# MrGiovanni/R-Super

Hardware: AMD Instinct MI355X
Metric: CT voxels/sec/node (96³ patch, bs=2/GPU) (higher is better)
Workload: dtype bf16; 1 GPU; R-Super 3D UNet(base 32, 26 classes, BasicBlock/IN) full training step (fwd + masked BCE + Dice loss + bwd + clip + AdamW + EMA), 96^3 patches, batch 2/GPU (BASELINE.json configs[1]); global_batch=2, patch=96, parallelism=dp1, sanity_checks_form=device-side flags read one step late (train_ddp.StepGuard)

## Files before the change

include/rsuper_hip.h:

```cpp
#ifndef RSUPER_HIP_H
#define RSUPER_HIP_H
#include <stddef.h>
#include <stdint.h>
#ifdef __cplusplus
extern "C" {
#endif

#define RSUPER_F32 0
#define RSUPER_BF16 1
#define RSUPER_OK 0
#define RSUPER_ERR_ARG 1
#define RSUPER_ERR_LAUNCH 2
#define RSUPER_ERR_UNSUPPORTED 3
#define RSUPER_ERR_NO_DEVICE 4

const char* rsuper_version(void);
int rsuper_device_check(void);


size_t rsuper_conv3_packed_elems(int dtype, int ka, int kb, int n_cols, int bn);

int rsuper_conv3_pack_weights(int dtype, int mode, const float* wa, const float* wb, int ka, int kb, int na, int nb,
                              int bn, void* packed, void* stream);

int rsuper_conv3_pack_weights_batch(int dtype, int n, const int* host_desc, const float* const* host_wa, const float* const* host_wb,
                                    const size_t* host_out_elems, void* packed, void* stream);

int rsuper_conv3_tiles(int D, int H, int W);

int rsuper_conv3_variant(int v);
int rsuper_conv3_wgrad2_min_tiles(int t);

int rsuper_conv3_plan(int dtype, int epi, int N, int D, int H, int W, int Ca, int Cb, int n_cols, int src_flags, int bn, int* plan);

int rsuper_conv3_box_bn(int dtype, int N, int D, int H, int W, int n_cols);

int rsuper_conv3_kd_bn(int dtype, int epi, int N, int D, int H, int W, int n_cols, int src_flags);

int rsuper_conv3_set_workspace(void* ptr, size_t bytes);
size_t rsuper_conv3_workspace_bytes(void);

int rsuper_conv3_part_rows(int dtype, int epi, int N, int D, int H, int W, int n_cols, int bn, int src_flags);

int rsuper_conv3_igemm(int dtype, int epi,
                       const void* xa, int lda, int Ca, const float* mra,
                       const void* xb, int ldb, int Cb, const float* mrb,
                       const void* packed, int n_cols, int bn, int N, int D, int H, int W,
                       void* out, int ldo, const void* res, int ldr, float* part,
                       const void* exa, int elda, int eCa, const float* emra,
                       const void* exb, int eldb, int eCb, const float* emrb, void* stream);
int rsuper_conv3_igemm_split_out(int dtype, int epi,
                                 const void* xa, int lda, int Ca, const float* mra,
                                 const void* xb, int ldb, int Cb, const float* mrb,
                                 const void* packed, int n_cols, int bn, int N, int D, int H, int W,
                                 void* out, int ldo, const void* res, int ldr, float* part,
                                 const void* exa, int elda, int eCa, const float* emra,
                                 const void* exb, int eldb, int eCb, const float* emrb, int out_split, long long out_part, void* stream);
int rsuper_conv3_s2_part_rows(int dtype, int mode, int Ca, int Cb, int n_cols, int N, int FD, int FH, int FW);
int rsuper_conv3_igemm_s2(int dtype, int mode, const void* xa, int lda, int Ca, const float* mra,
                          const void* xb, int ldb, int Cb, const void* packed, int n_cols, int N, int FD, int FH, int FW,
                          void* out, int ldo, float* part, const void* exa, int elda, const float* emra, void* stream);

int rsuper_conv3_wgrad_splits(int dtype, int Ca, int Cb, int Ya, int Yb, int N, int D, int H, int W);

// ... 219 lines not shown
```

r-super_amd/csrc/api.hip:

```cpp
#include <string.h>
#include <math.h>
#include <stdlib.h>
#include "common.hpp"
#include "kernels.hpp"
#include "misc.hpp"
#include "loss.hpp"
#include "morph.hpp"
#include "optim.hpp"
#include "../../include/rsuper_hip.h"

#define ST(s) ((hipStream_t)(s))

static inline bool dt_ok(int dt) { return dt == RS_F32 || dt == RS_BF16; }
static inline bool ch_ok(int C, int ld) { return C >= 0 && (C % 8) == 0 && (ld % 8) == 0 && ld >= C; }
static inline bool bn_ok(int bn) { return bn == 32 || bn == 64 || bn == 96 || bn == 128; }
static inline int ntiles_for(int n_cols, int bn) { const int per = bn / 32; return ((n_cols + bn - 1) / bn) * per; }
static inline int pack_cols(int mode, int na, int nb) { return mode == 1 ? (nb ? (nb & 0xFFFF) : na) : na + nb; }
static inline bool pack_range_ok(int mode, int na, int nb) { return mode != 1 || nb == 0 || ((nb >> 16) % 32 == 0 && (nb & 0xFFFF) > 0 && (nb >> 16) + (nb & 0xFFFF) <= na); }

#include "igemm_plan.hpp"

template <typename F>
static int for_chunks(int n, void* const* p, void* const* g, void* const* m, void* const* v, void* const* e, const size_t* numel, F f) {
    for (int i0 = 0; i0 < n; i0 += RS_MT_MAX) {
// ... 53 lines not shown
                                    const size_t* host_out_elems, void* packed, void* stream) {
    if (!dt_ok(dtype) || n <= 0 || !host_desc || !host_wa || !host_wb || !host_out_elems || !packed) return RS_ERR_ARG;
    const int KP = dtype == RS_F32 ? 4 : 8;
    for (int i0 = 0; i0 < n; i0 += RS_PACK_BATCH_MAX) {
        PackBatch b;
        memset(&b, 0, sizeof(b));
        b.n = n - i0 < RS_PACK_BATCH_MAX ? n - i0 : RS_PACK_BATCH_MAX;
        const size_t base = host_out_elems[i0];
        for (int i = 0; i < b.n; ++i) {
            const int* d = host_desc + (size_t)(i0 + i) * 6;
            if ((d[0] != 0 && d[0] != 1) || d[1] <= 0 || d[2] < 0 || d[3] <= 0 || d[4] < 0 || !bn_ok(d[5])) return RS_ERR_ARG;
            PackParams& q = b.q[i];
            q.wa = host_wa[i0 + i]; q.wb = host_wb[i0 + i]; q.mode = d[0]; q.ka = d[1]; q.kb = d[2]; q.na = d[3]; q.nb = d[4];
            if (!pack_range_ok(d[0], d[3], d[4])) return RS_ERR_ARG;
            q.ntiles = ntiles_for(pack_cols(d[0], d[3], d[4]), d[5]);
            if (!q.wa || ((host_out_elems[i0 + i] - base) % KP)) return RS_ERR_ARG;
            b.vec_start[i] = (host_out_elems[i0 + i] - base) / KP;
        }
        const int* dl = host_desc + (size_t)(i0 + b.n - 1) * 6;
        b.vec_start[b.n] = b.vec_start[b.n - 1] + rs_packed_elems(dtype, dl[1], dl[2], ntiles_for(pack_cols(dl[0], dl[3], dl[4]), dl[5])) / KP;
        for (int i = 0; i + 1 < b.n; ++i) {
            const int* d = host_desc + (size_t)(i0 + i) * 6;
            if (b.vec_start[i] + rs_packed_elems(dtype, d[1], d[2], ntiles_for(pack_cols(d[0], d[3], d[4]), d[5])) / KP != b.vec_start[i + 1]) return RS_ERR_ARG;
        }
        const int rc = rs_launch_pack_batch(b, dtype, (char*)packed + base * (dtype == RS_F32 ? 4 : 2), ST(stream));
        if (rc) return rc;
    }
    return RS_OK;
}

int rsuper_conv3_tiles(int D, int H, int W) { return ((D + 3) / 4) * ((H + 3) / 4) * ((W + 15) / 16); }

int rsuper_conv3_wgrad2_min_tiles(int t) { return rs_wgrad2_min_tiles(t); }

int rsuper_conv3_variant(int v) {
    if (v >= 0 && v <= 8 && v != 5) g_variant = v;
    return g_variant;
}
int rsuper_conv3_plan(int dtype, int epi, int N, int D, int H, int W, int Ca, int Cb, int n_cols, int src_flags, int bn, int* plan) {
    const IgemmPlan pl = igemm_plan(dtype, epi, N, D, H, W, Ca, Cb, n_cols, src_flags, bn);
    if (!plan || pl.kernel < 0) return RS_ERR_ARG;
    plan[0] = pl.kernel; plan[1] = pl.bn; plan[2] = pl.box_cfg; plan[3] = pl.nsplit; plan[4] = pl.part_rows;
    return RS_OK;
}
int rsuper_conv3_kd_bn(int dtype, int epi, int N, int D, int H, int W, int n_cols, int src_flags) {
    const IgemmPlan pl = igemm_plan(dtype, epi, N, D, H, W, 0, 0, n_cols, src_flags, 0);
    return pl.kernel == RS_IGEMM_KD ? pl.bn : 0;
}
int rsuper_conv3_box_bn(int dtype, int N, int D, int H, int W, int n_cols) {
    const IgemmPlan pl = igemm_plan(dtype, 0, N, D, H, W, 0, 0, n_cols, 1, 0);
    return pl.kernel == RS_IGEMM_BOX ? pl.bn : 0;
}
int rsuper_conv3_part_rows(int dtype, int epi, int N, int D, int H, int W, int n_cols, int bn, int src_flags) {
    return bn ? igemm_plan(dtype, epi, N, D, H, W, 0, 0, n_cols, src_flags, bn).part_rows : 0;
}

int rsuper_conv3_set_workspace(void* ptr, size_t bytes) {
    g_ws = ptr; g_ws_bytes = ptr ? bytes : 0;
    return RS_OK;
}
size_t rsuper_conv3_workspace_bytes(void) { return BOXC_WS_BYTES; }

int rsuper_conv3_s2_part_rows(int dtype, int mode, int Ca, int Cb, int n_cols, int N, int FD, int FH, int FW) {
    if ((mode != 1 && mode != 2) || FD <= 0 || FH <= 0 || FW <= 0 || N <= 0 || n_cols <= 0) return 0;
    const int OD = (FD + 1) / 2, OH = (FH + 1) / 2, OW = (FW + 1) / 2, td = mode == 2 ? 2 : 4;
    const S2Kernel k = s2_kernel(dtype, mode, Ca, Cb, n_cols, N, FD, FH, FW);
// ... 649 lines not shown
```

r-super_amd/csrc/conv3d_wgrad2.hip:

```cpp
#include "common.hpp"
#include "kernels.hpp"
#include "wgrad_frag.hpp"
#include <stdio.h>
#include <stdlib.h>
#include <type_traits>

namespace {

#ifdef WG2_PROF
__device__ unsigned long long g_wg2_prof[8 * 4];
#endif

constexpr int TD = 4, TH = 4, TW = 16, HD = TD + 2, HH = TH + 2, HW = TW + 2;
constexpr int XROWS = HD * HH * HW;
constexpr int XBYTES = XROWS * 64;
constexpr int YPLANE = 256 * 64;
constexpr int NT = 512, NW = 8;

__device__ __forceinline__ void dma16(const __amdgpu_buffer_rsrc_t& rs, uint32_t voff, uint32_t lds_byte) {
    asm volatile("s_mov_b32 m0, %1\n\ts_nop 0\n\tbuffer_load_dwordx4 %0, %2, 0 offen lds" : : "v"(voff), "s"(lds_byte), "s"(rs) : "memory", "m0");
}

constexpr bool pair_in_group(int G, int pidx) { return G < 3 ? pidx < 7 : pidx >= 7; }
constexpr bool unit_valid(int NDL, int dp, int hp, int pidx) {
    const int d = dp - pidx / 3, h = hp - pidx % 3;
    return d >= 0 && d < NDL && h >= 0 && h < TH;
}
constexpr int frag_uses(int G, int NDL, int dp, int hp) {
    int n = 0;
    for (int pidx = 0; pidx < 9; ++pidx) n += (pair_in_group(G, pidx) && unit_valid(NDL, dp, hp, pidx)) ? 1 : 0;
    return n;
}
struct Sched { int n; int dp[64], hp[64], kw[64]; };
constexpr Sched make_sched(int G, int NDL) {
    Sched s{};
    for (int dp = 0; dp < NDL + 2; ++dp)
        for (int hp = 0; hp < HH; ++hp) {
            if (frag_uses(G, NDL, dp, hp) == 0) continue;
            for (int kw = (G < 3 ? G : 0); kw <= (G < 3 ? G : 2); ++kw) { s.dp[s.n] = dp; s.hp[s.n] = hp; s.kw[s.n] = kw; ++s.n; }
        }
    return s;
}

template <int MT, int BD, bool NORM>
__global__ __launch_bounds__(NT, 2) void wgrad2_kernel(WgradParams p) {
    constexpr int NDL = MT == 2 ? 4 : 2;
    constexpr int BUF = XBYTES + MT * YPLANE;
    constexpr int NXV = (XROWS * 4 + NT - 1) / NT;
    constexpr int YK = 16 * MT / NW;
    constexpr int NV = NXV;
    extern __shared__ __attribute__((aligned(16))) char smem[];

    const int tid = threadIdx.x, lane = tid & 63;
    const int wave = __builtin_amdgcn_readfirstlane(tid >> 6);
    const int wsel = wave & 1, g = wave >> 1;
    const int dsel = MT == 1 ? wsel * 2 : 0;
    const int tiles_w = (p.W + TW - 1) / TW, tiles_h = (p.H + TH - 1) / TH, tiles_d = (p.D + TD - 1) / TD;
    const int tiles_per_sample = tiles_w * tiles_h * tiles_d;
    const WgBlockMap bm = wg_block_map(tiles_per_sample * p.N, p.splits);
    const int nchA = (p.xa.C + 31) / 32;
    const bool isB = bm.bx >= nchA;
    const ConvSrc& xs = isB ? p.xb : p.xa;
    const int c0 = (isB ? bm.bx - nchA : bm.bx) * 32;
    const int cin_total = p.xa.C + p.xb.C;
    const int cin_base = (isB ? p.xa.C : 0) + c0;
    const int Mtot = p.ya.C + p.yb.C;
    const int m0 = bm.by * MT * 32;
    constexpr bool norm = NORM;
    const int tiles = tiles_per_sample * p.N;

    const int x_off = dsel * (HH * HW * 64) + frag_lane_off<1>(64, lane);
    const int ya_off = XBYTES + (MT == 2 ? wsel * YPLANE : 0) + dsel * (TH * TW * 64) + frag_lane_off<1>(64, lane);

    const int s_slot = tid & 3, s_row = tid >> 2;
    const uint32_t nvox_total = (uint32_t)(p.N * p.D * p.H * p.W);
    const uint32_t xrowb = (uint32_t)xs.ld * 2u;
    const __amdgpu_buffer_rsrc_t xrs = __builtin_amdgcn_make_buffer_rsrc((void*)xs.x, 0, nvox_total * xrowb, 0x00020000);
    uint32_t xoffb[NXV], xpm[NXV];
    const bool x_cok = c0 + s_slot * 8 < xs.C;
#pragma unroll
    for (int i = 0; i < NXV; ++i) {
        const int r = s_row + 128 * i;
        const int hd = r / (HH * HW), rem = r - hd * (HH * HW);
        const int hh = rem / HW, hw = rem - hh * HW;
        xoffb[i] = (uint32_t)((hd * p.H + hh) * p.W + hw) * xrowb + (uint32_t)(c0 + s_slot * 8) * 2u;
        xpm[i] = (r < XROWS && x_cok) ? ((1u << hd) | (1u << (6 + hh)) | (1u << (12 + hw))) : (1u << 31);
    }
    const int x_st = s_row * 64 + s_slot * 16;
    const int prow = lane >> 2, pslot = lane & 3;
    __amdgpu_buffer_rsrc_t yrs[MT];
    uint32_t yrowb[MT], yoffb[MT];
    bool yok[MT];
#pragma unroll
    for (int q = 0; q < MT; ++q) {
        const int mq = m0 + 32 * q;
        const bool inA = mq < p.ya.C;
        const ConvSrc& ys = inA ? p.ya : p.yb;
        const int ch = (inA ? mq : mq - p.ya.C) + pslot * 8;
        yok[q] = mq < Mtot && ch < ys.C;
        yrowb[q] = (uint32_t)ys.ld * 2u;
        yoffb[q] = (uint32_t)prow * yrowb[q] + (uint32_t)ch * 2u;
        yrs[q] = __builtin_amdgcn_make_buffer_rsrc((void*)ys.x, 0, nvox_total * yrowb[q], 0x00020000);
    }
    const uint32_t lds0 = (uint32_t)(uintptr_t)(__attribute__((address_space(3))) char*)smem;
    const uint32_t ywbit = 1u << (8 + prow);

    const int tile0 = bm.tile0, tile_end = bm.tile_end, tstride = bm.tstride;

    struct IssueTile { uint32_t baseb, ybase; uint32_t xbad, ybad; int n; };
    uint4* dtab = (uint4*)(smem + 2 * BUF + p.N * 256);
    const int ntile = tile0 < tile_end ? (tile_end - 1 - tile0) / tstride + 1 : 0;
    for (int k = tid; k < ntile + 3; k += NT) {
        const bool live = k < ntile;
        const int q = live ? tile0 + k * tstride : 0;
        const int n = q / tiles_per_sample;
        int tw, th, td;
        rs_tile_coords(q - n * tiles_per_sample, tiles_w, tiles_h, tiles_d, tw, th, td);
        const int d0 = td * TD, h0 = th * TH, w0 = tw * TW;
        auto range = [](int o, int len, int nh) {
            const int lo = o >= 0 ? 0 : -o;
            int hi_ = len - 1 - o; if (hi_ > nh - 1) hi_ = nh - 1;
            return hi_ < lo ? 0u : (((2u << hi_) - 1u) & ~((1u << lo) - 1u));
        };
        const uint32_t xbad = live ? ~(range(d0 - 1, p.D, HD) | (range(h0 - 1, p.H, HH) << 6) | (range(w0 - 1, p.W, HW) << 12)) : 0xFFFFFFFFu;
        const uint32_t ybad = live ? (~(range(d0, p.D, TD) | (range(h0, p.H, TH) << 4) | (range(w0, p.W, TW) << 8)) & 0xFFFFFFu) : 0xFFFFFFu;
        dtab[k] = make_uint4((uint32_t)(((n * p.D + d0 - 1) * p.H + (h0 - 1)) * p.W + (w0 - 1)) * xrowb,
                             (uint32_t)(((n * p.D + d0) * p.H + h0) * p.W + w0), xbad, ybad | ((uint32_t)n << 24));
    }
    auto fetch_desc = [&](int k) {
        const uint4 v = dtab[k];
        IssueTile t;
        t.baseb = __builtin_amdgcn_readfirstlane(v.x); t.ybase = __builtin_amdgcn_readfirstlane(v.y);
        t.xbad = __builtin_amdgcn_readfirstlane(v.z);
        const uint32_t w = __builtin_amdgcn_readfirstlane(v.w);
        t.ybad = w & 0xFFFFFFu; t.n = (int)(w >> 24);
        return t;
    };
    uint4 px[NXV];
    auto ld16 = [&](const __amdgpu_buffer_rsrc_t& rs, uint32_t off) {
        const auto q = __builtin_amdgcn_raw_buffer_load_b128(rs, off, 0, 0);
        return make_uint4(q[0], q[1], q[2], q[3]);
    };
    auto issue_v = [&](const IssueTile& t, int i) {
        const bool ok = (xpm[i] & t.xbad) == 0u;
        px[i] = ld16(xrs, ok ? t.baseb + xoffb[i] : 0xFFFFFFF0u);
    };
    auto dma_y = [&](const IssueTile& t, int k, uint32_t buf) {
        const int y = wave + NW * k;
        const int q = MT == 1 ? 0 : (y >> 4), line = y & 15, d = line >> 2, h = line & 3;
        const uint32_t lbit = (1u << d) | (1u << (4 + h)) | ywbit;
        const bool ok = yok[q] && (lbit & t.ybad) == 0u;
        const uint32_t voff = ok ? (t.ybase + (uint32_t)((d * p.H + h) * p.W)) * yrowb[q] + yoffb[q] : 0xFFFFFFF0u;
        dma16(MT == 1 ? yrs[0] : (q ? yrs[MT - 1] : yrs[0]), voff, lds0 + buf + XBYTES + (uint32_t)y * 1024u);
    };
    float4* ntab = (float4*)(smem + 2 * BUF);
    if (norm) {
        for (int e = tid; e < p.N * 16; e += NT) {
            const int n = e >> 4, c = c0 + (e & 15) * 2;
            float4 v = make_float4(1.f, 1.f, 0.f, 0.f);
            if (c < xs.C) { const float* m = xs.mr + ((size_t)n * xs.C + c) * 2; v = make_float4(m[1], m[3], -m[0] * m[1], -m[2] * m[3]); }
            ntab[e] = v;
        }
    }
    const float4* nrow = ntab + s_slot * 4;
    float4 ncst[4];
    int cur_n = -1;
    auto load_norm = [&](int n) {
        if (!norm || n == cur_n) return;
        cur_n = n;
#pragma unroll
        for (int j = 0; j < 4; ++j) ncst[j] = nrow[16 * n + j];
    };
    auto commit_v = [&](char* buf, int i, const IssueTile& t) {
        {
            uint4 q = px[i];
            if (norm) {
                const uint32_t w[4] = {q.x, q.y, q.z, q.w};
                uint32_t o[4];
                const uint32_t m = (xpm[i] & t.xbad) == 0u ? 0xFFFFFFFFu : 0u;
#pragma unroll
                for (int j = 0; j < 4; ++j) {
                    const float4 c = ncst[j];
#ifndef WG2_PKFMA
                    float x0, x1;
                    asm("v_fma_f32 %0, %1, %2, %3" : "=v"(x0) : "v"(__uint_as_float(w[j] << 16)), "v"(c.x), "v"(c.z));
                    asm("v_fma_f32 %0, %1, %2, %3" : "=v"(x1) : "v"(__uint_as_float(w[j] & 0xffff0000u)), "v"(c.y), "v"(c.w));
                    i16x2_t v = __builtin_bit_cast(i16x2_t, f2bf2(x0, x1));
#else
                    f32x2_t x = {__uint_as_float(w[j] << 16), __uint_as_float(w[j] & 0xffff0000u)};
                    const f32x2_t s2 = {c.x, c.y}, b2 = {c.z, c.w};
                    x = __builtin_elementwise_fma(x, s2, b2);
                    i16x2_t v = __builtin_bit_cast(i16x2_t, f2bf2(x[0], x[1]));
#endif
                    const i16x2_t z = {0, 0};
                    v = __builtin_elementwise_max(v, z);
                    o[j] = __builtin_bit_cast(uint32_t, v) & m;
                }
                q = make_uint4(o[0], o[1], o[2], o[3]);
            }
            if (s_row + 128 * i < XROWS) *(uint4*)(buf + x_st + i * 8192) = q;
        }
    };

    auto run = [&](auto G_) {
        constexpr int G = std::remove_reference_t<decltype(G_)>::value;
        constexpr Sched S = make_sched(G, NDL);
        constexpr int KDMIN = G < 3 ? 0 : 2;
        constexpr int AP = NDL < 3 ? NDL : 3;
#ifndef WG2_HOOK_MODE
#define WG2_HOOK_MODE 1
#endif
        constexpr int HMODE = WG2_HOOK_MODE;
        constexpr bool late = HMODE == 0 ? false : ((G < 2) == (HMODE == 1));
        auto hook_step = [&](int i) constexpr { return HMODE == 0 ? (i * S.n) / NV : (late ? S.n / 2 : 0) + (i * (S.n / 2)) / NV; };
        f32x16_t acc[7];
#pragma unroll
        for (int i = 0; i < 7; ++i)
#pragma unroll
            for (int r = 0; r < 16; ++r) acc[i][r] = 0.f;

        __syncthreads();
        IssueTile t1 = fetch_desc(1);
        {
            const IssueTile t0 = fetch_desc(0);
#pragma unroll
            for (int k = 0; k < YK; ++k) dma_y(t0, k, 0);
#pragma unroll
            for (int i = 0; i < NV; ++i) issue_v(t0, i);
            load_norm(t0.n);
#pragma unroll
            for (int i = 0; i < NV; ++i) commit_v(smem, i, t0);
#pragma unroll
            for (int i = 0; i < NV; ++i) issue_v(t1, i);
        }
        asm volatile("s_waitcnt vmcnt(%0)" : : "n"(NV) : "memory");
        __syncthreads();

#ifdef WG2_PROF
        unsigned long long pf_loop = 0, pf_bar = 0;
#endif
        int it = 0;
        for (int tile = tile0; tile < tile_end; tile += tstride, ++it) {
#ifdef WG2_PROF
            const unsigned long long q0 = __builtin_readcyclecounter();
#endif
            const char* buf = smem + (it & 1) * BUF;
            char* nxt = smem + ((it + 1) & 1) * BUF;
            const IssueTile t2 = fetch_desc(it + 2);
            load_norm(t1.n);
#ifndef WG2_SKIP_STAGE
#pragma unroll
            for (int k = 0; k < YK; ++k) dma_y(t1, k, (uint32_t)((it + 1) & 1) * BUF);
#endif
            auto fetch_a = [&](int row) { return frag_bf16<1>(buf + ya_off + (row * TW) * 64, 64); };
            auto fetch_b = [&](int s) { return frag_bf16<1>(buf + x_off + ((S.dp[s] * HH + S.hp[s]) * HW + S.kw[s]) * 64, 64); };
            constexpr int BR = BD + 1;
            uint4 a[AP * TH], bq[BR];
#pragma unroll
            for (int h = 0; h < TH; ++h) a[h] = fetch_a(h);
#pragma unroll
            for (int s = 0; s < BD; ++s) bq[s] = fetch_b(s);
#pragma unroll
            for (int s = 0; s < S.n; ++s) {
#ifndef WG2_PRIO
#define WG2_PRIO 1
#endif
                if (WG2_PRIO == 1) {
                    if (s == 0) __builtin_amdgcn_s_setprio(3);
                    if (s == S.n / 4) __builtin_amdgcn_s_setprio(2);
                    if (s == S.n / 2) __builtin_amdgcn_s_setprio(1);
                    if (s == (3 * S.n) / 4) __builtin_amdgcn_s_setprio(0);
                }
                if (s + BD < S.n) bq[(s + BD) % BR] = fetch_b(s + BD);
                {
                    constexpr bool ring = AP < NDL;
                    const int pl = S.dp[s] - KDMIN + 1;
                    const bool first_of_plane = s == 0 || S.dp[s] != S.dp[s - 1];
                    const bool first_hp4 = S.hp[s] >= 4 && (s == 0 || S.dp[s] != S.dp[s - 1] || S.hp[s - 1] < 4);
                    if (pl >= 1 && pl < NDL && ((ring && G < 3) ? first_hp4 : first_of_plane)) {
#pragma unroll
                        for (int h = 0; h < TH; ++h) a[(pl % AP) * TH + h] = fetch_a(pl * TH + h);
                    }
                }
                __builtin_amdgcn_sched_barrier(0);
#pragma unroll
                for (int pidx = 0; pidx < 9; ++pidx) {
                    if (!pair_in_group(G, pidx) || !unit_valid(NDL, S.dp[s], S.hp[s], pidx)) continue;
                    const int d = S.dp[s] - pidx / 3, h = S.hp[s] - pidx % 3;
                    const int slot = G < 3 ? pidx : (pidx - 7) * 3 + S.kw[s];
#ifndef WG2_SKIP_MMA
                    mma32<bf16_t>(acc[slot], a[(d % AP) * TH + h], bq[s % BR]);
#else
                    if (s == 0) mma32<bf16_t>(acc[slot], a[(d % AP) * TH + h], bq[s % BR]);
#endif
                }
#ifndef WG2_SKIP_STAGE
#pragma unroll
                for (int i = 0; i < NV; ++i)
                    if (s == hook_step(i)) { commit_v(nxt, i, t1); issue_v(t2, i); }
#endif
                __builtin_amdgcn_sched_barrier(0);
            }
#ifdef WG2_PROF
            const unsigned long long q1 = __builtin_readcyclecounter();
#endif
#ifndef WG2_SKIP_STAGE
            asm volatile("s_waitcnt vmcnt(%0)" : : "n"(NV) : "memory");
#endif
            __syncthreads();
#ifdef WG2_PROF
            const unsigned long long q2 = __builtin_readcyclecounter();
            pf_loop += q1 - q0; pf_bar += q2 - q1;
#endif
            t1 = t2;
        }

#ifdef WG2_PROF
        if (blockIdx.x == 0 && blockIdx.y == 0 && blockIdx.z == 0 && lane == 0) { g_wg2_prof[wave * 4] = pf_loop; g_wg2_prof[wave * 4 + 1] = pf_bar; g_wg2_prof[wave * 4 + 2] = (unsigned long long)it; }
#endif
        if constexpr (MT == 1) {
            float* red = (float*)smem + (size_t)g * 7 * 16 * 64 + lane;
            if (wsel == 1) {
#pragma unroll
                for (int i = 0; i < 7; ++i)
#pragma unroll
                    for (int r = 0; r < 16; ++r) red[(i * 16 + r) * 64] = acc[i][r];
            }
            __syncthreads();
            if (wsel == 0) {
#pragma unroll
                for (int i = 0; i < 7; ++i)
#pragma unroll
                    for (int r = 0; r < 16; ++r) acc[i][r] += red[(i * 16 + r) * 64];
            }
        }
        if (MT == 2 || wsel == 0) {
            const int ci = c0 + (lane & 31);
            float* slab = p.ws + (size_t)bm.bz * 27 * Mtot * cin_total;
            const int mrow0 = m0 + (MT == 2 ? wsel * 32 : 0);
#pragma unroll
            for (int i = 0; i < (G < 3 ? 7 : 6); ++i) {
                const int tap = G < 3 ? i * 3 + G : 21 + i;
#pragma unroll
                for (int r = 0; r < 16; ++r) {
                    const int m = mrow0 + cd_row32(r, lane);
                    if (m < Mtot && ci < xs.C) slab[((size_t)tap * Mtot + m) * cin_total + cin_base + (lane & 31)] = acc[i][r];
                }
            }
        }
    };
    switch (g) {
        case 0: run(std::integral_constant<int, 0>{}); break;
        case 1: run(std::integral_constant<int, 1>{}); break;
        case 2: run(std::integral_constant<int, 2>{}); break;
        default: run(std::integral_constant<int, 3>{}); break;
    }
}

template <int MT, int BD, bool NORM>
int launch2(const WgradParams& p, hipStream_t st) {
    const int tiles = p.N * ((p.D + TD - 1) / TD) * ((p.H + TH - 1) / TH) * ((p.W + TW - 1) / TW);
    const int smem = 2 * (XBYTES + MT * YPLANE) + p.N * 256 + ((tiles + p.splits - 1) / p.splits + 4) * 16;
    if (smem > 160 * 1024) return RS_ERR_UNSUPPORTED;
    static_assert(MT == 2 || 4 * 7 * 16 * 64 * 4 <= 2 * (XBYTES + MT * YPLANE), "depth-half reduction scratch must fit the tile buffers");
    const int nch = (p.xa.C + 31) / 32 + (p.xb.C + 31) / 32;
    const int Mtot = p.ya.C + p.yb.C;
    dim3 grid(nch, (Mtot + MT * 32 - 1) / (MT * 32), p.splits), block(NT);
    auto k = wgrad2_kernel<MT, BD, NORM>;
    (void)hipFuncSetAttribute((const void*)k, hipFuncAttributeMaxDynamicSharedMemorySize, smem);
    hipLaunchKernelGGL(k, grid, block, smem, st, p);
#ifdef WG2_PROF
    if (getenv("RSUPER_WG2_PROF")) {
        unsigned long long h[32];
        (void)hipDeviceSynchronize();
        (void)hipMemcpyFromSymbol(h, HIP_SYMBOL(g_wg2_prof), sizeof(h));
        fprintf(stderr, "wg2_prof MT%d norm%d:", MT, (int)NORM);
        for (int w = 0; w < 8; ++w) fprintf(stderr, " w%d(g%d) loop %.0f bar %.0f |", w, w >> 1, (double)h[w * 4] / h[w * 4 + 2], (double)h[w * 4 + 1] / h[w * 4 + 2]);
        fprintf(stderr, " tiles %llu\n", h[2]);
    }
#endif
    return RS_OK;
}

}

bool rs_wgrad2_supported(const WgradParams& p, int dtype) {
    static const int off = getenv("RSUPER_WGRAD2") ? atoi(getenv("RSUPER_WGRAD2")) == 0 : 0;
    if (off || dtype != RS_BF16 || p.N > 32) return false;
    if (p.yb.C > 0 && (p.ya.C % 32)) return false;
    if ((p.xa.mr != nullptr) != (p.xb.C > 0 ? p.xb.mr != nullptr : p.xa.mr != nullptr)) return false;
    return true;
}

int rs_launch_wgrad2(const WgradParams& p, hipStream_t st) {
    const int Mtot = p.ya.C + p.yb.C;
#ifndef WG2_BD
#define WG2_BD 2
#endif
    const int tiles = p.N * ((p.D + TD - 1) / TD) * ((p.H + TH - 1) / TH) * ((p.W + TW - 1) / TW);
    const bool mt1 = Mtot <= 32 || rs_wgrad2_mt1(RS_BF16, Mtot, tiles);
    if (p.xa.mr) return mt1 ? launch2<1, WG2_BD, true>(p, st) : launch2<2, WG2_BD, true>(p, st);
    return mt1 ? launch2<1, WG2_BD, false>(p, st) : launch2<2, WG2_BD, false>(p, st);
}
```

r-super_amd/csrc/kernels.hpp:

```cpp
#pragma once
#include <hip/hip_runtime.h>
#include <stddef.h>
#include <stdint.h>

struct ConvSrc {
    const void* x;
    int ld;
    int C;
    const float* mr;
};

enum IgemmKernel {
    RS_IGEMM_CLASSIC = 0,
    RS_IGEMM_PC = 1,
    RS_IGEMM_WS = 2,
    RS_IGEMM_KD = 3,
    RS_IGEMM_BOX = 4
};

struct IgemmParams {
    ConvSrc a, b;
    const void* wp;
    int ntiles;
    int bn;
// ... 44 lines not shown
int rs_box_config(int N, int D, int H, int W, int n_cols);
int rs_box_part_rows(int cfg, int D, int H, int W);
int rs_box_nsplit(int N, int n_cols, int nch);
int rs_launch_igemm_box(const IgemmParams& p, int cfg, int epi, hipStream_t st);
int rs_launch_igemm_s2(const IgemmParams& p, int dtype, int mode, int FD, int FH, int FW, hipStream_t st);
bool rs_igemm_s2k_shape_ok(int dtype, int Ca, int Cb, int n_cols, int N, int FD, int FH, int FW);
int rs_igemm_s2k_part_rows(int ntiles, int n_cols, int N, int D, int H, int W);
int rs_launch_igemm_s2k(const IgemmParams& p, int FD, int FH, int FW, hipStream_t st);
bool rs_igemm_s2d_shape_ok(int dtype, int Ca, int Cb, int n_cols, int N, int FD, int FH, int FW);
int rs_igemm_s2d_part_rows(int n_cols, int N, int D, int H, int W);
int rs_launch_igemm_s2d(const IgemmParams& p, int FD, int FH, int FW, hipStream_t st);
size_t rs_packed_elems(int dtype, int ka, int kb, int ntiles);
int rs_launch_pack(const PackParams& q, int dtype, void* out, hipStream_t st);
int rs_token_attn_supported(int L, int Dh);
int rs_launch_token_attn(const float* qkv, float* o, float* p, const float* d_o, float* d_qkv, int B, int L, int H, int Dh, float scale, hipStream_t st);
int rs_launch_wgrad(const WgradParams& p, int dtype, int use_tr, hipStream_t st, bool reduce = true);
int rs_launch_wgrad_reduce(const WgradParams& p, hipStream_t st);
#define RS_REDUCE_BATCH_MAX 48
#define RS_REDUCE_STATS_MAX 2
struct ReduceBatch {
    int n;
    struct Entry { const float* ws; float* dwa; float* dwb; int splits, Mtot, Ya, Cin; unsigned blk_start; } e[RS_REDUCE_BATCH_MAX];
    unsigned blocks;
    int nstats;
    struct Stats { const float* part; float* out; int N, nblk, C, mode, split; float eps; double cnt; unsigned blk_start; } sj[RS_REDUCE_STATS_MAX];
};
int rs_launch_wgrad_reduce_batch(ReduceBatch& b, hipStream_t st);
bool rs_wgrad2_mt1(int dtype, int Mtot, int tiles_total);
int rs_wgrad_splits(int dtype, int Mtot, int nch, int tiles_total);
int rs_wgrad_sv_splits(int dtype, int Mtot, int Ya, int nch, int N, int D, int H, int W);
int rs_launch_wgrad_sv(const WgradParams& p, hipStream_t st);
bool rs_wgrad2_supported(const WgradParams& p, int dtype);
int rs_wgrad2_min_tiles(int t);
int rs_launch_wgrad2(const WgradParams& p, hipStream_t st);
int rs_wgrad_s2_splits(int dtype, int Ca, int Mtot, int N, int D, int H, int W);
int rs_launch_wgrad_s2(const WgradParams& p, int dtype, hipStream_t st);

size_t rs_pw_packed_bytes(int N, int K, int dtype);
int rs_launch_pointwise(int dtype, int mode, const float* x, int ldx, const float* w, const float* bias, const float* res, int ldr,
                        float* y, int ldy, int R, int K, int N, void* packed, hipStream_t st);
int rs_pw_wgrad_splits(int R, int N, int K);
int rs_launch_pointwise_pack_batch(int dtype, const long long* table, int n, long total_items, void* arena, hipStream_t st);
int rs_launch_pointwise_wgrad(int dtype, const float* dy, int ldy, const float* x, int ldx, int R, int N, int K, float* part, int S,
                              float* dw, float* db, hipStream_t st);
```

r-super_amd/csrc/wgrad_frag.hpp:

```cpp
#pragma once
#include "common.hpp"

typedef short v4s_t __attribute__((__vector_size__(4 * sizeof(short))));

struct WgBlockMap { int bx, by, bz, tile0, tile_end, tstride; };
__device__ __forceinline__ WgBlockMap wg_block_map(int tiles, int S) {
    const unsigned gx = gridDim.x, gy = gridDim.y, sib = gx * gy;
    WgBlockMap m;
    m.bx = (int)blockIdx.x; m.by = (int)blockIdx.y; m.bz = (int)blockIdx.z;
    if (S >= 8 && tiles >= 64) {
        const unsigned T = sib * (unsigned)S, L = blockIdx.x + gx * (blockIdx.y + gy * blockIdx.z);
        const unsigned q = T >> 3, r = T & 7;
        auto prefix = [&](unsigned x) { return x * q + (x < r ? x : r); };
        const unsigned V = prefix(L & 7) + (L >> 3);
        m.bx = (int)(V % gx); m.by = (int)((V / gx) % gy); m.bz = (int)(V / sib);
        const unsigned V0 = (unsigned)m.bz * sib;
        unsigned c = 0;
#pragma unroll
        for (unsigned x = 1; x < 8; ++x) c = V0 >= prefix(x) ? x : c;
        const unsigned zlo = (prefix(c) + sib - 1) / sib, zhi = (prefix(c + 1) + sib - 1) / sib;
        m.tile0 = (int)((long)tiles * zlo / S) + (m.bz - (int)zlo);
        m.tile_end = (int)((long)tiles * zhi / S);
        m.tstride = (int)(zhi - zlo);
    } else { m.tile0 = m.bz; m.tile_end = tiles; m.tstride = S; }
    return m;
}

template <int TR>
__device__ __forceinline__ int frag_lane_off(int pitch, int lane) {
    if (TR) {
        const int q = lane & 15, g = lane >> 4;
        return ((g >> 1) * 8 + (q >> 2)) * pitch + ((g & 1) * 16 + (q & 3) * 4) * 2;
    }
    return ((lane >> 5) * 8) * pitch + (lane & 31) * 2;
}
template <int TR>
__device__ __forceinline__ uint4 frag_bf16(const char* a, int pitch) {
    uint4 r;
    if (TR) {
        v4s_t lo = __builtin_amdgcn_ds_read_tr16_b64_v4i16((__attribute__((address_space(3))) v4s_t*)(a));
        v4s_t hi = __builtin_amdgcn_ds_read_tr16_b64_v4i16((__attribute__((address_space(3))) v4s_t*)(a + 4 * pitch));
        union { v4s_t v; uint2 u; } ul, uh;
        ul.v = lo; uh.v = hi;
        r = make_uint4(ul.u.x, ul.u.y, uh.u.x, uh.u.y);
    } else {
        uint32_t e[8];
#pragma unroll
        for (int j = 0; j < 8; ++j) e[j] = *(const bf16_t*)(a + j * pitch);
        r = make_uint4(e[0] | (e[1] << 16), e[2] | (e[3] << 16), e[4] | (e[5] << 16), e[6] | (e[7] << 16));
    }
    return r;
}
```

r-super_amd/hip/lib.py:

```python
import ctypes
import os
from ctypes import c_int, c_long, c_longlong, c_size_t, c_float, c_double, c_void_p, c_uint32, c_uint

_HERE = os.path.dirname(os.path.abspath(__file__))
SO_PATH = os.path.join(os.path.dirname(_HERE), 'csrc', 'librsuper_hip.so')

F32, BF16 = 0, 1
BLUR_MAX_RADIUS = 5
_LIB = None

P = c_void_p
_SIGS = {
    'rsuper_version': (ctypes.c_char_p, []),
    'rsuper_device_check': (c_int, []),
    'rsuper_conv3_packed_elems': (c_size_t, [c_int] * 5),
    'rsuper_conv3_pack_weights': (c_int, [c_int, c_int, P, P, c_int, c_int, c_int, c_int, c_int, P, P]),
    'rsuper_conv3_pack_weights_batch': (c_int, [c_int, c_int, P, P, P, P, P, P]),
    'rsuper_conv3_tiles': (c_int, [c_int] * 3),
    'rsuper_conv3_variant': (c_int, [c_int]),
    'rsuper_conv3_wgrad2_min_tiles': (c_int, [c_int]),
    'rsuper_conv3_plan': (c_int, [c_int] * 11 + [P]),
    'rsuper_conv3_box_bn': (c_int, [c_int] * 6),
    'rsuper_conv3_kd_bn': (c_int, [c_int] * 8),
    'rsuper_conv3_set_workspace': (c_int, [P, c_size_t]),
    'rsuper_conv3_workspace_bytes': (c_size_t, []),
    'rsuper_conv3_wgrad_splits': (c_int, [c_int] * 9),
    'rsuper_conv3_part_rows': (c_int, [c_int] * 9),
    'rsuper_conv3_s2_part_rows': (c_int, [c_int] * 9),
    'rsuper_conv3_igemm_s2': (c_int, [c_int, c_int, P, c_int, c_int, P, P, c_int, c_int, P, c_int, c_int, c_int, c_int, c_int, P, c_int, P, P, c_int, P, P]),
    'rsuper_conv3_igemm': (c_int, [c_int, c_int, P, c_int, c_int, P, P, c_int, c_int, P, P, c_int, c_int, c_int, c_int, c_int, c_int,
                                   P, c_int, P, c_int, P, P, c_int, c_int, P, P, c_int, c_int, P, P]),
    'rsuper_conv3_igemm_split_out': (c_int, [c_int, c_int, P, c_int, c_int, P, P, c_int, c_int, P, P, c_int, c_int, c_int, c_int, c_int, c_int,
                                             P, c_int, P, c_int, P, P, c_int, c_int, P, P, c_int, c_int, P, c_int, c_longlong, P]),
    'rsuper_conv3_wgrad': (c_int, [c_int, c_int, P, c_int, c_int, P, P, c_int, c_int, P, P, c_int, c_int, P, c_int, c_int,
                                   P, P, P, c_int, c_int, c_int, c_int, c_int, P]),
    'rsuper_conv3_wgrad_partial': (c_int, [c_int, c_int, P, c_int, c_int, P, P, c_int, c_int, P, P, c_int, c_int, P, c_int, c_int,
                                           P, c_int, c_int, c_int, c_int, c_int, P]),
    'rsuper_conv3_wgrad_reduce': (c_int, [P, c_int, c_int, c_int, c_int, P, P, P]),
    'rsuper_conv3_wgrad_reduce_batch': (c_int, [c_int, P, P, P, P, P, P, P, P]),
    'rsuper_conv3_wgrad_reduce_batch_stats': (c_int, [c_int, P, P, P, P, P, P, P, c_int, P, P, P, P, P, P, P, P, c_float, P]),
    'rsuper_conv3_wgrad_s2_splits': (c_int, [c_int] * 7),
    'rsuper_conv3_wgrad_s2': (c_int, [c_int, P, c_int, c_int, P, P, c_int, c_int, P, c_int, c_int, P, P, P, c_int, c_int, c_int, c_int, c_int, P]),
    'rsuper_pointwise_packed_bytes': (c_size_t, [c_int, c_int, c_int]),
    'rsuper_pointwise': (c_int, [c_int, c_int, P, c_int, P, P, P, c_int, P, c_int, c_long, c_int, c_int, P, P]),
    'rsuper_pointwise_pack_batch': (c_int, [c_int, P, c_int, c_long, P, P]),
    'rsuper_pointwise_wgrad_splits': (c_int, [c_long, c_int, c_int]),
    'rsuper_pointwise_wgrad': (c_int, [c_int, P, c_int, P, c_int, c_long, c_int, c_int, P, c_int, P, P, P]),
    'rsuper_stats_finalize': (c_int, [P, c_int, c_int, c_int, c_double, c_float, c_int, c_int, P, P]),
    'rsuper_glue_variant': (c_int, [c_int]),
    'rsuper_in_bwd_finalize': (c_int, [c_int, P, c_int, P, c_int, P, P, P, c_int, P, c_int, P, c_int, c_int, c_int, c_int, P]),
    'rsuper_maxpool2_fwd': (c_int, [c_int, P, c_int, P, c_int, P, c_int, c_int, c_int, c_int, c_int, c_int, P]),
    'rsuper_maxpool2_bwd': (c_int, [c_int, P, c_int, P, c_int, P, c_int, c_int, c_int, c_int, c_int, c_int, P]),
    'rsuper_maxpool2_bwd_add': (c_int, [c_int, P, c_int, P, c_int, P, c_int, P, c_int, c_int, c_int, c_int, c_int, c_int, P]),
# ... 133 lines not shown
```

Before: 168.2 million voxels/s.

## Add sliding depth-ring halo reuse to wgrad2 kernel for deep volumes

Adds a SLIDE variant of the wgrad2 weight-gradient kernel. Each block now processes contiguous depth-column runs of tiles, and the x halo is kept in an LDS ring of depth planes, so consecutive tiles along depth load only the new planes instead of the full 6-plane halo. This cuts redundant global loads and LDS stores of halo data. The cost is more complex tile scheduling, ring-slot address arithmetic and changed hook timing. It is enabled by default when the depth has enough tiles (12 or 24 depth tiles).

```diff
diff --git a/include/rsuper_hip.h b/include/rsuper_hip.h
--- a/include/rsuper_hip.h
+++ b/include/rsuper_hip.h
@@ -30,6 +30,7 @@
 
 int rsuper_conv3_variant(int v);
 int rsuper_conv3_wgrad2_min_tiles(int t);
+int rsuper_conv3_wgrad2_slide(int v);
 
 int rsuper_conv3_plan(int dtype, int epi, int N, int D, int H, int W, int Ca, int Cb, int n_cols, int src_flags, int bn, int* plan);
 
diff --git a/r-super_amd/csrc/api.hip b/r-super_amd/csrc/api.hip
--- a/r-super_amd/csrc/api.hip
+++ b/r-super_amd/csrc/api.hip
@@ -109,6 +109,7 @@
 int rsuper_conv3_tiles(int D, int H, int W) { return ((D + 3) / 4) * ((H + 3) / 4) * ((W + 15) / 16); }
 
 int rsuper_conv3_wgrad2_min_tiles(int t) { return rs_wgrad2_min_tiles(t); }
+int rsuper_conv3_wgrad2_slide(int v) { return rs_wgrad2_slide(v); }
 
 int rsuper_conv3_variant(int v) {
     if (v >= 0 && v <= 8 && v != 5) g_variant = v;
diff --git a/r-super_amd/csrc/conv3d_wgrad2.hip b/r-super_amd/csrc/conv3d_wgrad2.hip
--- a/r-super_amd/csrc/conv3d_wgrad2.hip
+++ b/r-super_amd/csrc/conv3d_wgrad2.hip
@@ -16,6 +16,10 @@
 constexpr int XBYTES = XROWS * 64;
 constexpr int YPLANE = 256 * 64;
 constexpr int NT = 512, NW = 8;
+constexpr int PLANEB = HH * HW * 64;
+constexpr int NSLOT = 2 * HD;
+constexpr int RING = NSLOT * PLANEB;
+static_assert(RING == 2 * XBYTES, "the ring takes exactly the bytes of the two halo buffers");
 
 __device__ __forceinline__ void dma16(const __amdgpu_buffer_rsrc_t& rs, uint32_t voff, uint32_t lds_byte) {
     asm volatile("s_mov_b32 m0, %1\n\ts_nop 0\n\tbuffer_load_dwordx4 %0, %2, 0 offen lds" : : "v"(voff), "s"(lds_byte), "s"(rs) : "memory", "m0");
@@ -42,7 +46,7 @@
     return s;
 }
 
-template <int MT, int BD, bool NORM>
+template <int MT, int BD, bool NORM, bool SLIDE>
 __global__ __launch_bounds__(NT, 2) void wgrad2_kernel(WgradParams p) {
     constexpr int NDL = MT == 2 ? 4 : 2;
     constexpr int BUF = XBYTES + MT * YPLANE;
@@ -69,8 +73,8 @@
     constexpr bool norm = NORM;
     const int tiles = tiles_per_sample * p.N;
 
-    const int x_off = dsel * (HH * HW * 64) + frag_lane_off<1>(64, lane);
-    const int ya_off = XBYTES + (MT == 2 ? wsel * YPLANE : 0) + dsel * (TH * TW * 64) + frag_lane_off<1>(64, lane);
+    const int x_off = (SLIDE ? 0 : dsel * (HH * HW * 64)) + frag_lane_off<1>(64, lane);
+    const int ya_off = (SLIDE ? 0 : XBYTES) + (MT == 2 ? wsel * YPLANE : 0) + dsel * (TH * TW * 64) + frag_lane_off<1>(64, lane);
 
     const int s_slot = tid & 3, s_row = tid >> 2;
     const uint32_t nvox_total = (uint32_t)(p.N * p.D * p.H * p.W);
@@ -105,17 +109,38 @@
     const uint32_t lds0 = (uint32_t)(uintptr_t)(__attribute__((address_space(3))) char*)smem;
     const uint32_t ywbit = 1u << (8 + prow);
 
-    const int tile0 = bm.tile0, tile_end = bm.tile_end, tstride = bm.tstride;
-
-    struct IssueTile { uint32_t baseb, ybase; uint32_t xbad, ybad; int n; };
+    int c1 = 0, run0 = 0, nslide = 0;
+    if constexpr (SLIDE) {
+        const int len = bm.r1 - bm.r0, per = bm.rn * tiles_d, c = len / per;
+        const int R0 = bm.r0 + c * per, Rlen = bm.r1 - R0;
+        c1 = c * tiles_d;
+        run0 = R0 + (int)((long)Rlen * bm.rj / bm.rn);
+        nslide = c1 + (R0 + (int)((long)Rlen * (bm.rj + 1) / bm.rn) - run0);
+    }
+    auto tile_of = [&](int k) {
+        if (k < c1) { const int i = k / tiles_d; return bm.r0 + (i * bm.rn + bm.rj) * tiles_d + (k - i * tiles_d); }
+        return run0 + (k - c1);
+    };
+    const int tile0 = SLIDE ? 0 : bm.tile0, tile_end = SLIDE ? nslide : bm.tile_end, tstride = SLIDE ? 1 : bm.tstride;
+
+    struct IssueTile { uint32_t baseb, ybase; uint32_t xbad, ybad; int n; uint32_t cont; };
     uint4* dtab = (uint4*)(smem + 2 * BUF + p.N * 256);
     const int ntile = tile0 < tile_end ? (tile_end - 1 - tile0) / tstride + 1 : 0;
     for (int k = tid; k < ntile + 3; k += NT) {
         const bool live = k < ntile;
-        const int q = live ? tile0 + k * tstride : 0;
+        const int q = live ? (SLIDE ? tile_of(k) : tile0 + k * tstride) : 0;
         const int n = q / tiles_per_sample;
         int tw, th, td;
-        rs_tile_coords(q - n * tiles_per_sample, tiles_w, tiles_h, tiles_d, tw, th, td);
+        bool cont = false;
+        if constexpr (SLIDE) {
+            const int rem = q - n * tiles_per_sample, col = rem / tiles_d;
+            int z;
+            rs_tile_coords(col, tiles_w, tiles_h, 1, tw, th, z);
+            td = rem - col * tiles_d;
+            cont = live && k > 0 && tile_of(k - 1) == q - 1 && td > 0 && (td + 1) * TD <= p.D;
+        } else {
+            rs_tile_coords(q - n * tiles_per_sample, tiles_w, tiles_h, tiles_d, tw, th, td);
+        }
         const int d0 = td * TD, h0 = th * TH, w0 = tw * TW;
         auto range = [](int o, int len, int nh) {
             const int lo = o >= 0 ? 0 : -o;
@@ -124,7 +149,10 @@
         };
         const uint32_t xbad = live ? ~(range(d0 - 1, p.D, HD) | (range(h0 - 1, p.H, HH) << 6) | (range(w0 - 1, p.W, HW) << 12)) : 0xFFFFFFFFu;
         const uint32_t ybad = live ? (~(range(d0, p.D, TD) | (range(h0, p.H, TH) << 4) | (range(w0, p.W, TW) << 8)) & 0xFFFFFFu) : 0xFFFFFFu;
-        dtab[k] = make_uint4((uint32_t)(((n * p.D + d0 - 1) * p.H + (h0 - 1)) * p.W + (w0 - 1)) * xrowb,
+        if (cont)
+            dtab[k] = make_uint4((uint32_t)(((n * p.D + d0 + 1) * p.H + (h0 - 1)) * p.W + (w0 - 1)) * xrowb,
+                                 (uint32_t)(((n * p.D + d0) * p.H + h0) * p.W + w0), (xbad & ~0x3Fu) | ((xbad & 0x3Fu) >> 2) | 0x30u, ybad | ((uint32_t)n << 24) | (1u << 31));
+        else dtab[k] = make_uint4((uint32_t)(((n * p.D + d0 - 1) * p.H + (h0 - 1)) * p.W + (w0 - 1)) * xrowb,
                              (uint32_t)(((n * p.D + d0) * p.H + h0) * p.W + w0), xbad, ybad | ((uint32_t)n << 24));
     }
     auto fetch_desc = [&](int k) {
@@ -133,7 +161,7 @@
         t.baseb = __builtin_amdgcn_readfirstlane(v.x); t.ybase = __builtin_amdgcn_readfirstlane(v.y);
         t.xbad = __builtin_amdgcn_readfirstlane(v.z);
         const uint32_t w = __builtin_amdgcn_readfirstlane(v.w);
-        t.ybad = w & 0xFFFFFFu; t.n = (int)(w >> 24);
+        t.ybad = w & 0xFFFFFFu; t.n = SLIDE ? (int)((w >> 24) & 0x7Fu) : (int)(w >> 24); t.cont = SLIDE ? w >> 31 : 0u;
         return t;
     };
     uint4 px[NXV];
@@ -145,13 +173,13 @@
         const bool ok = (xpm[i] & t.xbad) == 0u;
         px[i] = ld16(xrs, ok ? t.baseb + xoffb[i] : 0xFFFFFFF0u);
     };
-    auto dma_y = [&](const IssueTile& t, int k, uint32_t buf) {
+    auto dma_y = [&](const IssueTile& t, int k, uint32_t ybuf) {
         const int y = wave + NW * k;
         const int q = MT == 1 ? 0 : (y >> 4), line = y & 15, d = line >> 2, h = line & 3;
         const uint32_t lbit = (1u << d) | (1u << (4 + h)) | ywbit;
         const bool ok = yok[q] && (lbit & t.ybad) == 0u;
         const uint32_t voff = ok ? (t.ybase + (uint32_t)((d * p.H + h) * p.W)) * yrowb[q] + yoffb[q] : 0xFFFFFFF0u;
-        dma16(MT == 1 ? yrs[0] : (q ? yrs[MT - 1] : yrs[0]), voff, lds0 + buf + XBYTES + (uint32_t)y * 1024u);
+        dma16(MT == 1 ? yrs[0] : (q ? yrs[MT - 1] : yrs[0]), voff, lds0 + ybuf + (uint32_t)y * 1024u);
     };
     float4* ntab = (float4*)(smem + 2 * BUF);
     if (norm) {
@@ -171,7 +199,7 @@
 #pragma unroll
         for (int j = 0; j < 4; ++j) ncst[j] = nrow[16 * n + j];
     };
-    auto commit_v = [&](char* buf, int i, const IssueTile& t) {
+    auto norm_v = [&](int i, const IssueTile& t) {
         {
             uint4 q = px[i];
             if (norm) {
@@ -198,8 +226,20 @@
                 }
                 q = make_uint4(o[0], o[1], o[2], o[3]);
             }
-            if (s_row + 128 * i < XROWS) *(uint4*)(buf + x_st + i * 8192) = q;
-        }
+            return q;
+        }
+    };
+    auto commit_v = [&](char* buf, int i, const IssueTile& t) {
+        const uint4 q = norm_v(i, t);
+        if (s_row + 128 * i < XROWS) *(uint4*)(buf + x_st + i * 8192) = q;
+    };
+    static_assert(XROWS - 5 * 128 == 8 && 4 * (HH * HW) - 3 * 128 == 48, "row limits of the last vectors");
+    auto commit_s = [&](uint32_t wv, int i, const IssueTile& t) {
+        const uint4 q = norm_v(i, t);
+        uint32_t a = wv + (uint32_t)i * 8192u;
+        a = min(a, a - (uint32_t)RING);
+        const bool ok = i == 3 ? (!t.cont || s_row < 48) : (i == 5 ? s_row < 8 : true);
+        if (ok) *(uint4*)(smem + a) = q;
     };
 
     auto run = [&](auto G_) {
@@ -210,9 +250,15 @@
 #ifndef WG2_HOOK_MODE
 #define WG2_HOOK_MODE 1
 #endif
+#ifndef WG2_SLIDE_HOOKS
+#define WG2_SLIDE_HOOKS 1
+#endif
         constexpr int HMODE = WG2_HOOK_MODE;
         constexpr bool late = HMODE == 0 ? false : ((G < 2) == (HMODE == 1));
-        auto hook_step = [&](int i) constexpr { return HMODE == 0 ? (i * S.n) / NV : (late ? S.n / 2 : 0) + (i * (S.n / 2)) / NV; };
+        auto hook_step = [&](int i) constexpr {
+            if (SLIDE && HMODE != 0 && WG2_SLIDE_HOOKS) return (late ? S.n / 2 : 0) + (i < 4 ? (i * (S.n / 2)) / 4 : ((4 * (i - 4) + 1) * (S.n / 2)) / 8);
+            return HMODE == 0 ? (i * S.n) / NV : (late ? S.n / 2 : 0) + (i * (S.n / 2)) / NV;
+        };
         f32x16_t acc[7];
 #pragma unroll
         for (int i = 0; i < 7; ++i)
@@ -224,12 +270,15 @@
         {
             const IssueTile t0 = fetch_desc(0);
 #pragma unroll
-            for (int k = 0; k < YK; ++k) dma_y(t0, k, 0);
+            for (int k = 0; k < YK; ++k) dma_y(t0, k, SLIDE ? RING : XBYTES);
 #pragma unroll
             for (int i = 0; i < NV; ++i) issue_v(t0, i);
             load_norm(t0.n);
 #pragma unroll
-            for (int i = 0; i < NV; ++i) commit_v(smem, i, t0);
+            for (int i = 0; i < NV; ++i) {
+                if constexpr (SLIDE) commit_s((uint32_t)x_st, i, t0);
+                else commit_v(smem, i, t0);
+            }
 #pragma unroll
             for (int i = 0; i < NV; ++i) issue_v(t1, i);
         }
@@ -240,6 +289,7 @@
         unsigned long long pf_loop = 0, pf_bar = 0;
 #endif
         int it = 0;
+        int bslot = 0;
         for (int tile = tile0; tile < tile_end; tile += tstride, ++it) {
 #ifdef WG2_PROF
             const unsigned long long q0 = __builtin_readcyclecounter();
@@ -250,10 +300,30 @@
             load_norm(t1.n);
 #ifndef WG2_SKIP_STAGE
 #pragma unroll
-            for (int k = 0; k < YK; ++k) dma_y(t1, k, (uint32_t)((it + 1) & 1) * BUF);
-#endif
-            auto fetch_a = [&](int row) { return frag_bf16<1>(buf + ya_off + (row * TW) * 64, 64); };
-            auto fetch_b = [&](int s) { return frag_bf16<1>(buf + x_off + ((S.dp[s] * HH + S.hp[s]) * HW + S.kw[s]) * 64, 64); };
+            for (int k = 0; k < YK; ++k)
+                dma_y(t1, k, SLIDE ? (uint32_t)RING + (uint32_t)((it + 1) & 1) * (MT * YPLANE) : (uint32_t)((it + 1) & 1) * BUF + XBYTES);
+#endif
+            const char* ybuf = SLIDE ? smem + RING + (it & 1) * (MT * YPLANE) : buf;
+            const char* xpl[NDL + 2];
+            uint32_t wv = 0;
+            if constexpr (SLIDE) {
+#pragma unroll
+                for (int j = 0; j < NDL + 2; ++j) {
+                    int sl = bslot + dsel + j;
+                    sl = sl >= NSLOT ? sl - NSLOT : sl;
+                    xpl[j] = smem + x_off + sl * PLANEB;
+                }
+                int ws_ = bslot + HD;
+                ws_ = ws_ >= NSLOT ? ws_ - NSLOT : ws_;
+                wv = (uint32_t)(ws_ * PLANEB + x_st);
+                bslot += t1.cont ? TD : HD;
+                bslot = bslot >= NSLOT ? bslot - NSLOT : bslot;
+            }
+            auto fetch_a = [&](int row) { return frag_bf16<1>(ybuf + ya_off + (row * TW) * 64, 64); };
+            auto fetch_b = [&](int s) {
+                if constexpr (SLIDE) return frag_bf16<1>(xpl[S.dp[s]] + (S.hp[s] * HW + S.kw[s]) * 64, 64);
+                else return frag_bf16<1>(buf + x_off + ((S.dp[s] * HH + S.hp[s]) * HW + S.kw[s]) * 64, 64);
+            };
             constexpr int BR = BD + 1;
             uint4 a[AP * TH], bq[BR];
 #pragma unroll
@@ -297,7 +367,14 @@
 #ifndef WG2_SKIP_STAGE
 #pragma unroll
                 for (int i = 0; i < NV; ++i)
-                    if (s == hook_step(i)) { commit_v(nxt, i, t1); issue_v(t2, i); }
+                    if (s == hook_step(i)) {
+                        if constexpr (SLIDE) {
+                            const bool need = i < 3 ? true : (i == 3 ? (!t1.cont || wave < 3) : (i == 4 ? !t1.cont : (!t1.cont && wave == 0)));
+                            if (need) commit_s(wv, i, t1);
+                        }
+                        else commit_v(nxt, i, t1);
+                        issue_v(t2, i);
+                    }
 #endif
                 __builtin_amdgcn_sched_barrier(0);
             }
@@ -357,7 +434,7 @@
     }
 }
 
-template <int MT, int BD, bool NORM>
+template <int MT, int BD, bool NORM, bool SLIDE>
 int launch2(const WgradParams& p, hipStream_t st) {
     const int tiles = p.N * ((p.D + TD - 1) / TD) * ((p.H + TH - 1) / TH) * ((p.W + TW - 1) / TW);
     const int smem = 2 * (XBYTES + MT * YPLANE) + p.N * 256 + ((tiles + p.splits - 1) / p.splits + 4) * 16;
@@ -366,7 +443,7 @@
     const int nch = (p.xa.C + 31) / 32 + (p.xb.C + 31) / 32;
     const int Mtot = p.ya.C + p.yb.C;
     dim3 grid(nch, (Mtot + MT * 32 - 1) / (MT * 32), p.splits), block(NT);
-    auto k = wgrad2_kernel<MT, BD, NORM>;
+    auto k = wgrad2_kernel<MT, BD, NORM, SLIDE>;
     (void)hipFuncSetAttribute((const void*)k, hipFuncAttributeMaxDynamicSharedMemorySize, smem);
     hipLaunchKernelGGL(k, grid, block, smem, st, p);
 #ifdef WG2_PROF
@@ -374,7 +451,7 @@
         unsigned long long h[32];
         (void)hipDeviceSynchronize();
         (void)hipMemcpyFromSymbol(h, HIP_SYMBOL(g_wg2_prof), sizeof(h));
-        fprintf(stderr, "wg2_prof MT%d norm%d:", MT, (int)NORM);
+        fprintf(stderr, "wg2_prof MT%d norm%d slide%d:", MT, (int)NORM, (int)SLIDE);
         for (int w = 0; w < 8; ++w) fprintf(stderr, " w%d(g%d) loop %.0f bar %.0f |", w, w >> 1, (double)h[w * 4] / h[w * 4 + 2], (double)h[w * 4 + 1] / h[w * 4 + 2]);
         fprintf(stderr, " tiles %llu\n", h[2]);
     }
@@ -392,6 +469,18 @@
     return true;
 }
 
+int rs_wgrad2_slide(int v) {
+    static int mode = getenv("RSUPER_WG2_SLIDE") ? atoi(getenv("RSUPER_WG2_SLIDE")) : 1;
+    if (v >= 0) mode = v;
+    return mode;
+}
+static bool rs_wgrad2_slide_for(const WgradParams& p, bool mt1, int tiles) {
+    const int mode = rs_wgrad2_slide(-1);
+    if (mode != 1) return mode > 1;
+    (void)tiles;
+    return (p.D + TD - 1) / TD >= (mt1 ? 12 : 24);
+}
+
 int rs_launch_wgrad2(const WgradParams& p, hipStream_t st) {
     const int Mtot = p.ya.C + p.yb.C;
 #ifndef WG2_BD
@@ -399,6 +488,10 @@
 #endif
     const int tiles = p.N * ((p.D + TD - 1) / TD) * ((p.H + TH - 1) / TH) * ((p.W + TW - 1) / TW);
     const bool mt1 = Mtot <= 32 || rs_wgrad2_mt1(RS_BF16, Mtot, tiles);
-    if (p.xa.mr) return mt1 ? launch2<1, WG2_BD, true>(p, st) : launch2<2, WG2_BD, true>(p, st);
-    return mt1 ? launch2<1, WG2_BD, false>(p, st) : launch2<2, WG2_BD, false>(p, st);
-}
+    if (rs_wgrad2_slide_for(p, mt1, tiles)) {
+        if (p.xa.mr) return mt1 ? launch2<1, WG2_BD, true, true>(p, st) : launch2<2, WG2_BD, true, true>(p, st);
+        return mt1 ? launch2<1, WG2_BD, false, true>(p, st) : launch2<2, WG2_BD, false, true>(p, st);
+    }
+    if (p.xa.mr) return mt1 ? launch2<1, WG2_BD, true, false>(p, st) : launch2<2, WG2_BD, true, false>(p, st);
+    return mt1 ? launch2<1, WG2_BD, false, false>(p, st) : launch2<2, WG2_BD, false, false>(p, st);
+}
diff --git a/r-super_amd/csrc/kernels.hpp b/r-super_amd/csrc/kernels.hpp
--- a/r-super_amd/csrc/kernels.hpp
+++ b/r-super_amd/csrc/kernels.hpp
@@ -100,6 +100,7 @@
 int rs_launch_wgrad_sv(const WgradParams& p, hipStream_t st);
 bool rs_wgrad2_supported(const WgradParams& p, int dtype);
 int rs_wgrad2_min_tiles(int t);
+int rs_wgrad2_slide(int v);
 int rs_launch_wgrad2(const WgradParams& p, hipStream_t st);
 int rs_wgrad_s2_splits(int dtype, int Ca, int Mtot, int N, int D, int H, int W);
 int rs_launch_wgrad_s2(const WgradParams& p, int dtype, hipStream_t st);
diff --git a/r-super_amd/csrc/wgrad_frag.hpp b/r-super_amd/csrc/wgrad_frag.hpp
--- a/r-super_amd/csrc/wgrad_frag.hpp
+++ b/r-super_amd/csrc/wgrad_frag.hpp
@@ -3,7 +3,7 @@
 
 typedef short v4s_t __attribute__((__vector_size__(4 * sizeof(short))));
 
-struct WgBlockMap { int bx, by, bz, tile0, tile_end, tstride; };
+struct WgBlockMap { int bx, by, bz, tile0, tile_end, tstride, r0, r1, rj, rn; };
 __device__ __forceinline__ WgBlockMap wg_block_map(int tiles, int S) {
     const unsigned gx = gridDim.x, gy = gridDim.y, sib = gx * gy;
     WgBlockMap m;
@@ -22,7 +22,8 @@
         m.tile0 = (int)((long)tiles * zlo / S) + (m.bz - (int)zlo);
         m.tile_end = (int)((long)tiles * zhi / S);
         m.tstride = (int)(zhi - zlo);
-    } else { m.tile0 = m.bz; m.tile_end = tiles; m.tstride = S; }
+        m.r0 = (int)((long)tiles * zlo / S); m.r1 = m.tile_end; m.rj = m.bz - (int)zlo; m.rn = m.tstride;
+    } else { m.tile0 = m.bz; m.tile_end = tiles; m.tstride = S; m.r0 = 0; m.r1 = tiles; m.rj = m.bz; m.rn = S; }
     return m;
 }
 
diff --git a/r-super_amd/hip/lib.py b/r-super_amd/hip/lib.py
--- a/r-super_amd/hip/lib.py
+++ b/r-super_amd/hip/lib.py
@@ -19,6 +19,7 @@
     'rsuper_conv3_tiles': (c_int, [c_int] * 3),
     'rsuper_conv3_variant': (c_int, [c_int]),
     'rsuper_conv3_wgrad2_min_tiles': (c_int, [c_int]),
+    'rsuper_conv3_wgrad2_slide': (c_int, [c_int]),
     'rsuper_conv3_plan': (c_int, [c_int] * 11 + [P]),
     'rsuper_conv3_box_bn': (c_int, [c_int] * 6),
     'rsuper_conv3_kd_bn': (c_int, [c_int] * 8),
```

Result: no change. 168.8 million voxels/s, median of 6 (+0.4%).
